# B3zaleel/draco-sharp

Hardware: NVIDIA B200
Metric: decoded points/sec (higher is better)
Workload: dtype i32->f32

## Files before the change

### draco_sharp_b200/csrc/dcb_device.cuh

```cuda
#pragma once
#include <cuda_runtime.h>
#include <stdint.h>

#include "dcb_internal.h"
#include "dcb_kernels.h"

namespace dcb {

__device__ __forceinline__ int32_t zigzag_dec(uint32_t v) {
  return (int32_t)((v >> 1) ^ (0u - (v & 1u)));
}

__device__ __forceinline__ int32_t wrap_original(int32_t pred, int32_t corr, int32_t mn, int32_t mx, int32_t max_diff) {
  pred = pred > mx ? mx : (pred < mn ? mn : pred);
  int32_t o = (int32_t)((uint32_t)pred + (uint32_t)corr);
  if (o > mx)
    o = (int32_t)((uint32_t)o - (uint32_t)max_diff);
  else if (o < mn)
    o = (int32_t)((uint32_t)o + (uint32_t)max_diff);
  return o;
}

__device__ __forceinline__ int32_t wrap_regular(int32_t pred, int32_t corr, int32_t mn, int32_t mx, int32_t max_diff) {
  int32_t o = (int32_t)((uint32_t)pred + (uint32_t)corr);
// ... 203 lines not shown
#define DCB_RING_BYTES 128u
#endif

__device__ __forceinline__ void cp_async16(uint32_t smem_addr, const void *gsrc) {
  asm volatile("cp.async.ca.shared.global [%0], [%1], 16;\n" ::"r"(smem_addr), "l"(gsrc) : "memory");
}
__device__ __forceinline__ void cp_async_commit() { asm volatile("cp.async.commit_group;\n" ::: "memory"); }
template <int N>
__device__ __forceinline__ void cp_async_wait() {
  asm volatile("cp.async.wait_group %0;\n" ::"n"(N) : "memory");
}
__device__ __forceinline__ uint32_t lds_u32(uint32_t a) {
  uint32_t v;
  asm volatile("ld.shared.u32 %0, [%1];\n" : "=r"(v) : "r"(a));
  return v;
}

struct TableGeom {
  uint32_t lut_bytes;
  uint32_t lutb_bytes;
  uint32_t blk_bytes;
  uint32_t ent_bytes;
  uint32_t cap_entries;
  uint32_t cap_exc;
  uint32_t lut_shift;
  uint32_t compact;
  uint32_t zig;
  uint32_t direct_prec;
  uint32_t direct;
};

template <typename T, bool GLOBAL>
struct RansLane {
  uint32_t x;
  uint32_t p1;
  uint32_t L, L8, L16, mask, prec_bits;
  uint32_t lut_base;
  uint32_t lut_mask, lut_sh;
  uint32_t ring;
  uint32_t ent_off;
  uint32_t val_delta;
  uint32_t dprefix;
  uint32_t t_split, a_sh, a_mask, b_base, base_b;
  uint32_t lutb_addr;
  uint32_t blk_addr;
  uint32_t blk_mask;
  uint32_t cum_addr;
  uint32_t n_entries_tab;
  bool split_ok;
  uint32_t max_abs_val;
  uint32_t d_freq, d_off, d_ent;
  const uint8_t *ent0;
  const uint8_t *lut0;
  const uint8_t *arena;
  int64_t end;
  uint32_t p1_init;
  uint32_t off_init;
  int64_t loaded_lo;

  __device__ __forceinline__ uint32_t consumed() const { return p1_init - p1; }
  __device__ __forceinline__ uint32_t bytes_left() const { return off_init - consumed(); }

  template <int MAX_CHUNKS>
  __device__ __forceinline__ void top_up() {
    const int64_t ptr = end - (int64_t)consumed();
    const int64_t floor_lo = ((ptr + 15) & ~15ll) - (int64_t)DCB_RING_BYTES;
#pragma unroll
    for (int k = 0; k < MAX_CHUNKS; ++k) {
      if (loaded_lo - 16 >= floor_lo) {
        loaded_lo -= 16;
        cp_async16(ring | ((uint32_t)loaded_lo & (DCB_RING_BYTES - 1u)), arena + loaded_lo);
      }
    }
    cp_async_commit();
  }

  uint32_t pk_hi, pk_lo, pk_sh;
  __device__ __forceinline__ void prefetch() {
    pk_hi = lds_u32(ring | (p1 & (DCB_RING_BYTES - 4u)));
    pk_lo = lds_u32(ring | ((p1 + DCB_RING_BYTES - 4u) & (DCB_RING_BYTES - 4u)));
    pk_sh = (p1 & 3u) * 8u + 8u;
  }
  __device__ __forceinline__ uint32_t peek() const { return __funnelshift_rc(pk_lo, pk_hi, pk_sh); }

  __device__ __forceinline__ uint32_t lut_load(uint32_t xx) const {
    const uint32_t a = lut_base | ((xx >> lut_sh) & lut_mask);
    if (GLOBAL) return *reinterpret_cast<const T *>(lut0 + a);
    uint32_t v;
    if (sizeof(T) == 2) asm volatile("ld.shared.u16 %0, [%1];\n" : "=r"(v) : "r"(a));
    else asm volatile("ld.shared.u32 %0, [%1];\n" : "=r"(v) : "r"(a));
    return v;
  }

  template <bool CAREFUL, int PROBE>
  __device__ __forceinline__ uint32_t step() {
    const uint32_t v = peek();
    uint32_t sh;
    if (sizeof(T) == 2 && !GLOBAL) {
      const uint32_t sh2 = x < L8 ? 16u : 8u;
      sh = x < L ? sh2 : 0u;
    } else {
      const uint32_t sh3 = x < L16 ? 24u : 16u;
      const uint32_t sh2 = x < L8 ? sh3 : 8u;
      sh = x < L ? sh2 : 0u;
    }
    if (CAREFUL) sh = min(sh, 8u * bytes_left());
    const uint32_t xr = __funnelshift_l(v, x, sh);
    p1 -= sh >> 3;
    prefetch();
    const uint32_t r = xr & mask;
    const uint32_t q = xr >> prec_bits;
    uint32_t o, c0, c1, c2;
    if (PROBE == 2) {
      const uint32_t r2 = r << 1;
      uint32_t f, off;
      asm volatile("ld.shared.u16 %0, [%1];\n" : "=r"(f) : "r"(d_freq + r2));
      asm volatile("ld.shared.u16 %0, [%1];\n" : "=r"(off) : "r"(d_off + r2));
      asm volatile("ld.shared.u16 %0, [%1];\n" : "=r"(o) : "r"(d_ent + r2));
      x = q * f + off;
      return o;
    }
    if (PROBE == 1) {
      const uint32_t a_a = ((xr >> a_sh) & a_mask) | lut_base;
      const uint32_t a_b = (r >> 1) + b_base;
      const uint32_t a = r >= t_split ? a_b : a_a;
      const uint32_t a_k = ((xr >> 5) & blk_mask) | blk_addr;
// ... 113 lines not shown
    const uint32_t rank2 = ca - cum_addr;
    if (rank2 >= 2u * dprefix) {
      int32_t v;
      asm volatile("ld.shared.s16 %0, [%1];\n" : "=r"(v) : "r"(ca + val_delta));
      return v;
    }
    return zigzag_dec(rank2 >> 1);
  }

  __device__ __forceinline__ uint32_t value_at_plain(uint32_t ca, bool compact) const {
    const uint32_t rank2 = ca - cum_addr;
    if (compact && rank2 >= 2u * dprefix) {
      uint32_t v;
      asm volatile("ld.shared.u16 %0, [%1];\n" : "=r"(v) : "r"(ca + val_delta));
      return v;
    }
    return rank2 >> 1;
  }

  __device__ __forceinline__ int32_t value(uint32_t o, bool compact, bool zig) const {
    const uint32_t rank = (o - ent_off) / (uint32_t)sizeof(T);
    if (compact && rank >= dprefix) {
      if (sizeof(T) == 2) {
        return zig ? (int32_t) * reinterpret_cast<const int16_t *>(ent0 + o + val_delta)
                   : (int32_t) * reinterpret_cast<const uint16_t *>(ent0 + o + val_delta);
      }
      return *reinterpret_cast<const int32_t *>(ent0 + o + val_delta);
    }
    return zig ? zigzag_dec(rank) : (int32_t)rank;
  }
  __device__ __forceinline__ uint32_t symbol(uint32_t o, const TableGeom &g) const {
    const int32_t v = value(o, g.compact != 0, g.zig != 0);
    if (!g.zig) return (uint32_t)v;
    return v >= 0 ? ((uint32_t)v << 1) : ((((uint32_t)(-(v + 1))) << 1) | 1u);
  }

  __device__ int init_state(const uint8_t *arena_, const StreamDesc &d) {
    const uint64_t n = d.payload_len;
    if (n < 1) return DCB_ERR_RANS_INIT;
    const uint8_t *p = arena_ + d.payload_off;
    const uint32_t tag = (uint32_t)p[n - 1] >> 6;
    if (n < tag + 1) return DCB_ERR_RANS_INIT;
    uint32_t v = 0;
    for (uint32_t i = 0; i <= tag; ++i) v |= (uint32_t)p[n - 1 - tag + i] << (8 * i);
    v &= (tag == 0) ? 0x3Fu : (tag == 1) ? 0x3FFFu : (tag == 2) ? 0x3FFFFFu : 0x3FFFFFFFu;
    prec_bits = d.prec_bits;
    L = 4u << d.prec_bits;
    L8 = L >> 8;
    L16 = L >> 16;
    mask = (1u << d.prec_bits) - 1u;
    x = v + L;
    if (x >= L * 256u) return DCB_ERR_RANS_INIT;
    off_init = (uint32_t)(n - (tag + 1));
    arena = arena_;
    end = (int64_t)(d.payload_off + off_init);
    p1_init = (uint32_t)end - 1u;
    p1 = p1_init;
    loaded_lo = (end + 15) & ~15ll;
    return DCB_OK;
  }
  __device__ __forceinline__ void init_ring(uint32_t ring_addr) {
    ring = ring_addr;
    top_up<DCB_RING_BYTES / 16>();
    cp_async_wait<0>();
    prefetch();
  }

  __device__ int build(const uint8_t *arena_, const StreamDesc &d, const TableGeom &g, T *ent, uint32_t ent_off_) {
    ent_off = ent_off_;
    lut_sh = g.lut_shift - (sizeof(T) == 2 ? 1u : 2u);
    lut_mask = g.lut_bytes - (uint32_t)sizeof(T);
    split_ok = false;
    T *cum = ent;
    T *val = ent + g.cap_entries + 2u;
    uint64_t pos = d.table_off;
    const uint64_t bend = d.buf_end;
    for (int i = 0; i < 10; ++i) {
      if (pos >= bend) return DCB_ERR_EOF;
      if (!(arena_[pos++] & 0x80)) break;
    }
    const uint32_t ns = d.num_symbols;
    const uint32_t prec = 1u << d.prec_bits;
    if (!g.compact && ns > g.cap_entries) return DCB_ERR_TABLE;
    dprefix = g.compact ? 0xFFFFFFFFu : 0u;
    uint64_t c = 0;
    uint32_t ne = 0;
    bool overflow = false;
    uint32_t last_sym = 0;
    for (uint32_t i = 0; i < ns; ++i) {
      if (pos >= bend) return DCB_ERR_EOF;
      const uint32_t pd = arena_[pos++];
      const uint32_t token = pd & 3u;
      if (token == 3u) {
        const uint32_t off = pd >> 2;
        if (i + off >= ns) return DCB_ERR_TABLE;
        if (!g.compact)
          for (uint32_t j = 0; j <= off; ++j) cum[i + j] = (T)(c > prec ? prec : c);
        i += off;
      } else {
        uint32_t prob = pd >> 2;
        for (uint32_t b = 0; b < token; ++b) {
          if (pos >= bend) return DCB_ERR_EOF;
          prob |= (uint32_t)arena_[pos++] << (8 * (b + 1) - 2);
        }
        if (prob) last_sym = i;
        if (g.compact) {
          if (prob) {
            if (c + prob > prec || ne >= g.cap_entries) overflow = true;
            if (!overflow) {
              if (dprefix == 0xFFFFFFFFu && i != ne) dprefix = ne;
              if (dprefix != 0xFFFFFFFFu) {
// ... 116 lines not shown
    if (g.direct) a = (a + 15u) & ~15u;
    else a = (a + g.lut_bytes - 1u) & ~(g.lut_bytes - 1u);
    l.lut0 = a - base_addr;
    a += lanes * g.lut_bytes;
  } else {
    l.lut0 = 0;
  }
  a = (a + DCB_RING_BYTES - 1u) & ~(DCB_RING_BYTES - 1u);
  l.ring0 = a - base_addr;
  a += lanes * DCB_RING_BYTES;
  l.blk0 = l.lutb0 = a - base_addr;
  if (!table_global && g.lutb_bytes) {
    a = (a + g.blk_bytes - 1u) & ~(g.blk_bytes - 1u);
    l.blk0 = a - base_addr;
    a += lanes * g.blk_bytes;
    l.lutb0 = a - base_addr;
    a += (lanes * g.lutb_bytes + 15u) & ~15u;
  }
  l.ent0 = a - base_addr;
  return l;
}

template <int NCP, typename T, bool TG, bool DUMP, int MODE, int TAB, bool CAREFUL, int PROBE>
__device__ __forceinline__ void decode_entry(RansLane<T, TG> &rl, const TableGeom &g, const PostParams &pp, int32_t *prev,
                                             int32_t *v, int32_t *dptr, uint32_t dump, uint64_t e) {
#pragma unroll
  for (int c = 0; c < NCP; ++c) {
    const uint32_t o = rl.template step<CAREFUL, PROBE>();
    const bool compact = TAB == 0 ? g.compact != 0 : TAB == 2;
    const bool zig = MODE == 0 ? g.zig != 0 : MODE != 3;
    v[c] = rl.value(o, compact, zig);
    if (DUMP && (dump & DCB_DUMP_SYMBOLS)) dptr[e * NCP + c] = (int32_t)rl.symbol(o, g);
  }
  const int recon = recon_of<MODE>(pp);
  if (recon == RECON_DELTA_WRAP) {
#pragma unroll
    for (int c = 0; c < NCP; ++c) {
      prev[c] = wrap_original(prev[c], v[c], pp.mn, pp.mx, pp.max_diff);
      v[c] = prev[c];
    }
  } else if (recon == RECON_DELTA_OCT || recon == RECON_DELTA_OCT_CANON) {
    if (NCP == 2) {
      oct_original(pp.box, recon == RECON_DELTA_OCT_CANON, prev[0], prev[NCP - 1], v[0], v[NCP - 1]);
      v[0] = prev[0];
      v[NCP - 1] = prev[NCP - 1];
    }
  }
  if (DUMP && MODE != 3 && (dump & DCB_DUMP_QINTS)) {
#pragma unroll
    for (int c = 0; c < NCP; ++c) dptr[e * NCP + c] = v[c];
  }
}

template <int NCP, int MODE, bool LAST, int PROBE, bool COMPACT>
__device__ __forceinline__ void lean_sp_group(RansLane<uint16_t, false> &rl, const PostParams &pp, uint8_t *optr, uint32_t g,
                                              int32_t *prev, uint32_t &ca_prev, uint32_t &gate, uint32_t zero) {
  constexpr int kSyms = 4 * NCP;
  float f[kSyms];
  int32_t v[4][NCP];
#pragma unroll
  for (int s = 1; s <= kSyms; ++s) {
    uint32_t ca = 0;
    if (!(LAST && s == kSyms)) {
      const int sp = s % kSyms;
      if (sp % 3 == 0) rl.window_open();
      if (PROBE == 2) ca = (sp % 3 == 0) ? rl.template step_lean_direct<true>(gate, zero) : rl.template step_lean_direct<false>(gate, zero);
      else ca = (sp % 3 == 0) ? rl.template step_lean<true, true>(gate, zero) : rl.template step_lean<false, true>(gate, zero);
      if (sp % 3 == 2 || sp == kSyms - 1) rl.window_close();
    }
    const int c = (s - 1) % NCP;
    const int32_t corr = COMPACT ? rl.value_at(ca_prev) : zigzag_dec((ca_prev - rl.cum_addr) >> 1);
    if (MODE == 3 || MODE == 4) prev[c] = corr;
    else prev[c] = wrap_regular(prev[c], corr, pp.mn, pp.mx, pp.max_diff);
    if (MODE == 1) {
      f[s - 1] = pp.dequant(prev[c], c);
      gate = __float_as_uint(f[s - 1]);
    } else {
      v[(s - 1) / NCP][c] = prev[c];
      gate = (uint32_t)corr;
    }
    ca_prev = ca;
  }
  if (MODE == 1) {
    float4 *o = reinterpret_cast<float4 *>(reinterpret_cast<float *>(optr) + (uint64_t)g * kSyms);
#pragma unroll
    for (int k = 0; k < NCP; ++k) o[k] = make_float4(f[4 * k], f[4 * k + 1], f[4 * k + 2], f[4 * k + 3]);
  } else {
    store_group4<NCP>(pp, store_of<MODE>(pp), dsize_of<MODE>(pp), optr, (uint64_t)g * 4, v);
  }
}

template <bool LAST, int PROBE>
__device__ __forceinline__ void tag_sp_group(RansLane<uint16_t, false> &rl, bool compact, uint32_t *t, uint32_t &ca_prev,
                                             uint32_t &gate, uint32_t zero) {
#pragma unroll
  for (int s = 1; s <= 16; ++s) {
    uint32_t ca = 0;
    if (!(LAST && s == 16)) {
      const int sp = s % 16;
      if (sp % 3 == 0) rl.window_open();
      if (PROBE == 2) ca = (sp % 3 == 0) ? rl.template step_lean_direct<true>(gate, zero) : rl.template step_lean_direct<false>(gate, zero);
      else ca = (sp % 3 == 0) ? rl.template step_lean<true, true>(gate, zero) : rl.template step_lean<false, true>(gate, zero);
      if (sp % 3 == 2 || sp == 15) rl.window_close();
    }
    t[s - 1] = rl.value_at_plain(ca_prev, compact) & 0xFFu;
    gate = t[s - 1];
    ca_prev = ca;
  }
}

template <int PROBE>
__device__ __forceinline__ void run_tags_sp(RansLane<uint16_t, false> &rl, const TableGeom &geom, StreamDesc *dp, uint8_t *aux,
                                            uint32_t zero) {
  const StreamDesc &d = *dp;
  const uint32_t n_entries = d.n_entries;
  const uint32_t ncp = d.ncp;
  const uint64_t avail_bits = (d.buf_end - d.bits_off) * 8ull;
  uint8_t *tags = aux + d.tag_off;
  uint64_t *chunk_bits = reinterpret_cast<uint64_t *>(aux + d.tag_off + (((uint64_t)n_entries + 15ull) & ~15ull));
  const bool compact = geom.compact != 0;
  int status = DCB_OK;
  uint64_t bits = 0;
  uint32_t e = 0;
  if (n_entries >= 16u && rl.bytes_left() >= 48u) {
    rl.window_open();
    uint32_t ca_prev = PROBE == 2 ? rl.template step_lean_direct<true>(0u, zero) : rl.template step_lean<true>();
    uint32_t gate = 0;
    for (;;) {
      const bool last = !(e + 32u <= n_entries && rl.bytes_left() >= 96u);
      if ((e & (DCB_TAG_CHUNK - 1u)) == 0) chunk_bits[e / DCB_TAG_CHUNK] = bits;
      uint32_t t[16];
      if (last) tag_sp_group<true, PROBE>(rl, compact, t, ca_prev, gate, zero);
      else tag_sp_group<false, PROBE>(rl, compact, t, ca_prev, gate, zero);
      uint32_t tmax = 0, tsum = 0;
#pragma unroll
      for (int j = 0; j < 16; ++j) {
        tmax = max(tmax, t[j]);
        tsum += t[j];
      }
      const uint64_t nbits = bits + (uint64_t)tsum * ncp;
      if (tmax > 32u || nbits > avail_bits) {
// ... 45 lines not shown
```

### draco_sharp_b200/csrc/dcb_kernels.cu

```cuda
#include <cuda_runtime.h>
#include <stdint.h>
#include <algorithm>
#include <stdio.h>
#include <stdlib.h>

#include "dcb_device.cuh"
#include "dcb_internal.h"
#include "dcb_kernels.h"
#include "dcb_walk.h"

using namespace dcb;

namespace {

template <int NCP, typename T, bool DUMP, bool TG, int MODE, int TAB, bool SPLIT>
__device__ __forceinline__ void run_tail(RansLane<T, TG> &rl, const TableGeom &geom, const PostParams &pp, uint8_t *optr,
                                         int32_t *dptr, uint32_t dump, uint32_t n_entries, uint32_t g, int32_t *prev);

template <int NCP, typename T, bool DUMP, bool TG, int MODE, int TAB, bool SPLIT>
__device__ __forceinline__ void run_stream(RansLane<T, TG> &rl, const TableGeom &geom, const PostParams &pp, uint8_t *optr,
                                           int32_t *dptr, uint32_t dump, uint32_t n_entries, uint32_t g_min) {
  const int store = store_of<MODE>(pp), dsize = dsize_of<MODE>(pp);
  int32_t prev[NCP];
#pragma unroll
// ... 8 lines not shown
      decode_entry<NCP, T, TG, DUMP, MODE, TAB, false, SPLIT>(rl, geom, pp, prev, v[j], dptr, dump, (uint64_t)g * 4 + j);
    store_group4<NCP>(pp, store, dsize, optr, (uint64_t)g * 4, v);
    rl.template top_up<(kGroupBytes + 15) / 16 + 1>();
    cp_async_wait<1>();
  }
  run_tail<NCP, T, DUMP, TG, MODE, TAB, SPLIT>(rl, geom, pp, optr, dptr, dump, n_entries, g, prev);
}

template <int NCP, typename T, bool DUMP, bool TG, int MODE, int TAB, bool SPLIT>
__device__ __forceinline__ void run_tail(RansLane<T, TG> &rl, const TableGeom &geom, const PostParams &pp, uint8_t *optr,
                                         int32_t *dptr, uint32_t dump, uint32_t n_entries, uint32_t g, int32_t *prev) {
  const int store = store_of<MODE>(pp), dsize = dsize_of<MODE>(pp);
  for (uint32_t e = g * 4u; e < n_entries; ++e) {
    int32_t v[NCP];
    decode_entry<NCP, T, TG, DUMP, MODE, TAB, true, SPLIT>(rl, geom, pp, prev, v, dptr, dump, e);
    store_entry<NCP>(pp, store, dsize, optr, e, v);
    rl.template top_up<(3 * NCP + 15) / 16 + 1>();
    cp_async_wait<0>();
  }
}

template <int NCP, int MODE>
__device__ __forceinline__ void run_stream_lean(RansLane<uint16_t, false> &rl, const TableGeom &geom, const PostParams &pp,
                                                uint8_t *optr, uint32_t n_entries, uint32_t g_min) {
  const int store = store_of<MODE>(pp), dsize = dsize_of<MODE>(pp);
  int32_t prev[NCP];
  const int32_t p0 = 0 > pp.mx ? pp.mx : (0 < pp.mn ? pp.mn : 0);
#pragma unroll
  for (int c = 0; c < NCP; ++c) prev[c] = p0;
  constexpr uint32_t kGroupBytes = 4u * NCP * 3u;
  constexpr int kSyms = 4 * NCP;
  uint32_t g = 0;
  for (; g < g_min; ++g) {
    if (rl.bytes_left() < kGroupBytes) break;
    int32_t v[4][NCP];
#pragma unroll
    for (int s = 0; s < kSyms; ++s) {
      if (s % 3 == 0) rl.window_open();
      const uint32_t ca = (s % 3 == 0) ? rl.template step_lean<true>() : rl.template step_lean<false>();
      if (s % 3 == 2 || s == kSyms - 1) rl.window_close();
      const int32_t corr = rl.value_at(ca);
      const int c = s % NCP;
      prev[c] = wrap_regular(prev[c], corr, pp.mn, pp.mx, pp.max_diff);
      v[s / NCP][c] = prev[c];
    }
    store_group4<NCP>(pp, store, dsize, optr, (uint64_t)g * 4, v);
    rl.template top_up<(kGroupBytes + 15) / 16 + 1>();
    cp_async_wait<1>();
  }
  rl.prefetch();
  run_tail<NCP, uint16_t, false, false, MODE, 2, true>(rl, geom, pp, optr, nullptr, 0u, n_entries, g, prev);
}

template <int NCP, int MODE>
__device__ __forceinline__ void run_stream_lean_sp(RansLane<uint16_t, false> &rl, const TableGeom &geom, const PostParams &pp,
                                                   uint8_t *optr, uint32_t n_entries, uint32_t g_min, uint32_t zero) {
  int32_t prev[NCP];
  const int32_t p0 = 0 > pp.mx ? pp.mx : (0 < pp.mn ? pp.mn : 0);
#pragma unroll
  for (int c = 0; c < NCP; ++c) prev[c] = p0;
  constexpr uint32_t kGroupBytes = 4u * NCP * 3u;
  uint32_t g = 0;
  if (g_min > 0 && rl.bytes_left() >= kGroupBytes) {
    rl.window_open();
    uint32_t ca_prev = rl.template step_lean<true>();
    uint32_t gate = 0;
    while (g + 1 < g_min && rl.bytes_left() >= 2u * kGroupBytes + 4u) {
      lean_sp_group<NCP, MODE, false, 1, true>(rl, pp, optr, g, prev, ca_prev, gate, zero);
      ++g;
      rl.template top_up<(kGroupBytes + 15) / 16 + 1>();
      cp_async_wait<1>();
    }
    lean_sp_group<NCP, MODE, true, 1, true>(rl, pp, optr, g, prev, ca_prev, gate, zero);
    ++g;
    rl.template top_up<(kGroupBytes + 15) / 16 + 1>();
    cp_async_wait<1>();
  }
  rl.prefetch();
  run_tail<NCP, uint16_t, false, false, MODE, 2, true>(rl, geom, pp, optr, nullptr, 0u, n_entries, g, prev);
}

template <int NCP, typename T, bool DUMP, bool TABLE_GLOBAL, int MODE, int TAB>
__global__ void __launch_bounds__(32) rans_raw_fused_kernel(const uint8_t *__restrict__ arena, StreamDesc *streams,
                                                            const uint32_t *__restrict__ order, uint32_t n_streams,
                                                            uint32_t lanes, TableGeom geom, uint8_t *__restrict__ out,
                                                            uint8_t *__restrict__ dbg, uint8_t *__restrict__ aux,
                                                            uint8_t *__restrict__ tab_arena, uint32_t dump) {
  extern __shared__ __align__(16) uint8_t smem[];
  const uint32_t lane = threadIdx.x;
  const uint32_t slot = blockIdx.x * lanes + lane;
  const bool have = lane < lanes && slot < n_streams;
  StreamDesc *dp = have ? &streams[order[slot]] : nullptr;
  const uint32_t smem_base = (uint32_t)__cvta_generic_to_shared(smem);
  const SmemLayout lay = smem_layout(smem_base, lanes, geom, TABLE_GLOBAL);

  RansLane<T, TABLE_GLOBAL> rl;
  uint32_t n_entries = 0;
  T *lut = nullptr, *ent = nullptr;
  uint8_t *lutb = nullptr;
  uint32_t *blk = nullptr;
  bool split_ok = true;
  bool lean_ok = true;
  if (have) {
    const StreamDesc &d = *dp;
    n_entries = d.n_entries;
    if (NCP == 1 && MODE == 0 && d.ncp > 4) n_entries *= d.ncp;
    int status = DCB_OK;
    if (n_entries > 0) {
      uint32_t ent_off;
      if (TABLE_GLOBAL) {
        const uint32_t n_slots = gridDim.x * lanes;
        rl.lut0 = tab_arena;
        rl.ent0 = tab_arena + (size_t)n_slots * geom.lut_bytes;
        rl.lut_base = slot * geom.lut_bytes;
        ent_off = slot * geom.ent_bytes;
        lut = reinterpret_cast<T *>(tab_arena + (size_t)slot * geom.lut_bytes);
        ent = reinterpret_cast<T *>(const_cast<uint8_t *>(rl.ent0) + (size_t)slot * geom.ent_bytes);
      } else {
        rl.lut0 = nullptr;
        rl.ent0 = smem + lay.ent0;
        rl.lut_base = smem_base + lay.lut0 + lane * geom.lut_bytes;
        rl.lutb_addr = smem_base + lay.lutb0 + lane * geom.lutb_bytes;
        rl.blk_addr = smem_base + lay.blk0 + lane * geom.blk_bytes;
        blk = reinterpret_cast<uint32_t *>(smem + lay.blk0 + (size_t)lane * geom.blk_bytes);
        ent_off = lane * geom.ent_bytes;
        rl.cum_addr = smem_base + lay.ent0 + ent_off;
        lut = reinterpret_cast<T *>(smem + lay.lut0 + (size_t)lane * geom.lut_bytes);
        lutb = smem + lay.lutb0 + (size_t)lane * geom.lutb_bytes;
        ent = reinterpret_cast<T *>(smem + lay.ent0 + (size_t)lane * geom.ent_bytes);
      }
      status = rl.build(arena, d, geom, ent, ent_off);
      if (status == DCB_OK) status = rl.init_state(arena, d);
      if (status == DCB_OK) split_ok = rl.split_ok && !(dump & 0x80000000u);
      if (status == DCB_OK) {
        const int64_t md = 1ll + (int64_t)d.xf_b - (int64_t)d.xf_a;
        lean_ok = split_ok && geom.zig != 0 && !(dump & 0x40000000u) &&
                  (MODE == 3 || MODE == 4 ||
                   ((int64_t)rl.max_abs_val < md && d.xf_a >= -(1 << 29) && d.xf_b <= (1 << 29)));
      }
    }
    if (status != DCB_OK) {
      dp->status = status;
      n_entries = 0;
    }
  }
  const bool use_split = __all_sync(0xffffffffu, split_ok);
  const bool use_lean = __all_sync(0xffffffffu, lean_ok);
  uint32_t g_min = n_entries ? (n_entries >> 2) : 0xFFFFFFFFu;
#pragma unroll
  for (int o = 16; o > 0; o >>= 1) g_min = min(g_min, __shfl_xor_sync(0xffffffffu, g_min, o));
  if (n_entries == 0) return;
  rl.fill_lut(geom, lut, lutb, blk, ent, use_split);
  rl.init_ring(smem_base + lay.ring0 + lane * DCB_RING_BYTES);

  PostParams pp;
  pp.load(*dp);
  uint8_t *optr = out + dp->out_off;
  int32_t *dptr = DUMP ? reinterpret_cast<int32_t *>(dbg + dp->dbg_off) : nullptr;
  const bool wide_nc = NCP == 1 && MODE == 0 && dp->ncp > 4;
  if (wide_nc) {
    pp.recon = RECON_NONE;
    dump &= ~(uint32_t)DCB_DUMP_QINTS;
  }
  if (MODE == 3 || MODE == 4 || (MODE == 0 && (pp.recon == RECON_PARA_WRAP || pp.store == STORE_OCT_UNIT || wide_nc))) {
    optr = aux + dp->aux_off;
    if (NCP == 2 && pp.store == STORE_OCT_UNIT) {
      pp.recon = RECON_NONE;
      dump &= ~(uint32_t)DCB_DUMP_QINTS;
    }
    pp.store = STORE_NARROW;
    pp.dsize = 4;
  }
  if constexpr (sizeof(T) == 2 && !TABLE_GLOBAL && !DUMP && MODE >= 1 && MODE <= 4 && TAB == 2) {
    if (use_lean) {
#ifndef DCB_NO_LEAN_SP
      run_stream_lean_sp<NCP, MODE>(rl, geom, pp, optr, n_entries, g_min, blockIdx.y);
      return;
#endif
      if constexpr (MODE == 1 || MODE == 2) {
        run_stream_lean<NCP, MODE>(rl, geom, pp, optr, n_entries, g_min);
        return;
      }
    }
  }
  if (use_split)
    run_stream<NCP, T, DUMP, TABLE_GLOBAL, MODE, TAB, true>(rl, geom, pp, optr, dptr, dump, n_entries, g_min);
  else
    run_stream<NCP, T, DUMP, TABLE_GLOBAL, MODE, TAB, false>(rl, geom, pp, optr, dptr, dump, n_entries, g_min);
}

template <bool SPLIT>
__device__ __forceinline__ void run_tags(RansLane<uint16_t, false> &rl, const TableGeom &geom, StreamDesc *dp, uint8_t *aux) {
  const StreamDesc &d = *dp;
  const uint32_t n_entries = d.n_entries;
  const uint32_t ncp = d.ncp;
  const uint64_t avail_bits = (d.buf_end - d.bits_off) * 8ull;
  uint8_t *tags = aux + d.tag_off;
  uint64_t *chunk_bits = reinterpret_cast<uint64_t *>(aux + d.tag_off + (((uint64_t)n_entries + 15ull) & ~15ull));
  const bool compact = geom.compact != 0;
  int status = DCB_OK;
  uint64_t bits = 0;
  uint32_t e = 0;
  for (; e + 16 <= n_entries; e += 16) {
    if (rl.bytes_left() < 48u) break;
    if ((e & (DCB_TAG_CHUNK - 1u)) == 0) chunk_bits[e / DCB_TAG_CHUNK] = bits;
    uint32_t t[16];
#pragma unroll
    for (int j = 0; j < 16; ++j)
      t[j] = (uint32_t)rl.value(rl.template step<false, SPLIT>(), compact, false) & 0xFFu;
    uint32_t tmax = 0, tsum = 0;
#pragma unroll
    for (int j = 0; j < 16; ++j) {
      tmax = max(tmax, t[j]);
      tsum += t[j];
    }
    const uint64_t nbits = bits + (uint64_t)tsum * ncp;
    if (tmax > 32u || nbits > avail_bits) {
      for (int j = 0; j < 16 && status == DCB_OK; ++j) {
        if (t[j] > 32u) status = DCB_ERR_TAG;
        else {
          bits += (uint64_t)t[j] * ncp;
          if (bits > avail_bits) status = DCB_ERR_EOF;
        }
      }
      break;
    }
    uint4 pk;
    pk.x = t[0] | (t[1] << 8) | (t[2] << 16) | (t[3] << 24);
    pk.y = t[4] | (t[5] << 8) | (t[6] << 16) | (t[7] << 24);
// ... 486 lines not shown
      float x, y, z;
      oct_to_unit(q.x, q.y, scale, x, y, z);
      o[3ull * e] = x;
      o[3ull * e + 1] = y;
      o[3ull * e + 2] = z;
    }
  }
}

__global__ void copy_kernel(const uint8_t *__restrict__ arena, StreamDesc *streams, const uint32_t *__restrict__ order,
                            uint32_t n_streams, uint8_t *__restrict__ out) {
  for (uint32_t si = blockIdx.y; si < n_streams; si += gridDim.y) {
    const StreamDesc &d = streams[order[si]];
    if (d.status != DCB_OK) continue;
    const uint8_t *src = arena + d.raw_off;
    uint8_t *dst = out + d.out_off;
    for (uint64_t i = (uint64_t)blockIdx.x * blockDim.x + threadIdx.x; i < d.out_bytes; i += (uint64_t)gridDim.x * blockDim.x)
      dst[i] = src[i];
  }
}

}

static TableGeom geom_of(const RansLaunch &p) {
  TableGeom g{};
  g.lut_bytes = p.lut_bytes;
  g.lutb_bytes = p.lutb_bytes;
  g.blk_bytes = p.lutb_bytes ? (((1u << p.prec_bits) >> 7) << 2) : 0u;
  if (g.blk_bytes && g.blk_bytes < 16u) g.blk_bytes = 16u;
  g.ent_bytes = p.ent_bytes;
  g.cap_entries = p.cap_entries;
  g.cap_exc = p.cap_exc;
  g.lut_shift = p.lut_shift;
  g.compact = p.compact;
  g.zig = p.zig;
  return g;
}

uint32_t dcb_rans_smem_bytes(const RansLaunch &p, bool table_global) {
  uint32_t b = DCB_RING_BYTES + p.lanes_per_warp * DCB_RING_BYTES;
  if (!table_global && p.direct) return b + 32u + p.lanes_per_warp * (p.lut_bytes + p.ent_bytes);
  if (!table_global) {
    const uint32_t blk = p.lutb_bytes ? std::max(16u, ((1u << p.prec_bits) >> 7) << 2) : 0u;
    b += p.lut_bytes + blk + 16u + p.lanes_per_warp * (p.lut_bytes + p.lutb_bytes + blk + p.ent_bytes);
  }
  return b;
}

static uint32_t no_split_bit() {
  static const uint32_t bit = (getenv("DCB_NO_SPLIT") ? 0x80000000u : 0u) | (getenv("DCB_NO_LEAN") ? 0x40000000u : 0u);
  return bit;
}

template <int NCP, typename T, bool DUMP, bool TG, int MODE, int TAB = 0>
static cudaError_t launch_raw_t(const RansLaunch &p, const DevArenas &a, cudaStream_t st) {
  auto k = rans_raw_fused_kernel<NCP, T, DUMP, TG, MODE, TAB>;
  const uint32_t smem_bytes = dcb_rans_smem_bytes(p, TG);
  if (smem_bytes > 48 * 1024) {
    cudaError_t e = cudaFuncSetAttribute(k, cudaFuncAttributeMaxDynamicSharedMemorySize, (int)smem_bytes);
    if (e != cudaSuccess) return e;
  }
  cudaFuncSetAttribute(k, cudaFuncAttributePreferredSharedMemoryCarveout, (int)cudaSharedmemCarveoutMaxShared);
  const uint32_t grid = (p.n_streams + p.lanes_per_warp - 1) / p.lanes_per_warp;
  k<<<grid, 32, smem_bytes, st>>>(a.in, p.d_streams, p.d_order, p.n_streams, p.lanes_per_warp, geom_of(p), a.out, a.dbg,
                                  a.aux, a.tab, p.dump | no_split_bit());
  return cudaGetLastError();
}

template <int NCP, typename T>
static cudaError_t launch_raw_n(const RansLaunch &p, bool table_global, const DevArenas &a, cudaStream_t st) {
  const bool dump = p.dump != 0;
  if (table_global)
    return dump ? launch_raw_t<NCP, T, true, true, 0>(p, a, st) : launch_raw_t<NCP, T, false, true, 0>(p, a, st);
  return dump ? launch_raw_t<NCP, T, true, false, 0>(p, a, st) : launch_raw_t<NCP, T, false, false, 0>(p, a, st);
}

cudaError_t dcb_launch_rans_raw(const RansLaunch &p, int ncp, bool wide, bool table_global, const DevArenas &a,
                                cudaStream_t st) {
#ifdef DCB_DEV_ONLY_C2
  return launch_raw_t<3, uint16_t, false, false, 1, 2>(p, a, st);
#else
  if (!wide && !table_global && !p.dump) {
#define DCB_SPEC(M, N)                                                                           \
  if (p.mode == M && ncp == N)                                                                   \
    return p.compact ? launch_raw_t<N, uint16_t, false, false, M, 2>(p, a, st)                   \
                     : launch_raw_t<N, uint16_t, false, false, M, 1>(p, a, st);
    DCB_SPEC(1, 3)
    DCB_SPEC(1, 2)
    DCB_SPEC(2, 3)
    DCB_SPEC(2, 4)
    DCB_SPEC(3, 2)
    DCB_SPEC(4, 3)
    DCB_SPEC(4, 2)
#undef DCB_SPEC
  }
#define DCB_CASE(N)                                                       \
  case N:                                                                 \
    return wide ? launch_raw_n<N, uint32_t>(p, table_global, a, st)       \
                : launch_raw_n<N, uint16_t>(p, table_global, a, st);
  switch (ncp) {
    DCB_CASE(1)
    DCB_CASE(2)
    DCB_CASE(3)
    DCB_CASE(4)
    default:
      return cudaErrorInvalidValue;
  }
#undef DCB_CASE
#endif
}

cudaError_t dcb_launch_rans_tag(const RansLaunch &p, const DevArenas &a, cudaStream_t st) {
  const uint32_t smem_bytes = dcb_rans_smem_bytes(p, false);
  if (smem_bytes > 48 * 1024) {
    cudaError_t e = cudaFuncSetAttribute(rans_tag_kernel, cudaFuncAttributeMaxDynamicSharedMemorySize, (int)smem_bytes);
    if (e != cudaSuccess) return e;
  }
  cudaFuncSetAttribute(rans_tag_kernel, cudaFuncAttributePreferredSharedMemoryCarveout, (int)cudaSharedmemCarveoutMaxShared);
  const uint32_t grid = (p.n_streams + p.lanes_per_warp - 1) / p.lanes_per_warp;
  rans_tag_kernel<<<grid, 32, smem_bytes, st>>>(a.in, p.d_streams, p.d_order, p.n_streams, p.lanes_per_warp, geom_of(p),
                                                a.aux);
  return cudaGetLastError();
}

cudaError_t dcb_launch_wide_post(StreamDesc *d_streams, const uint32_t *d_order, uint32_t n, uint32_t dump, const DevArenas &a,
                                 cudaStream_t st) {
  if (n == 0) return cudaSuccess;
  const uint32_t grid = (n + 31) / 32;
  if (dump)
    wide_post_kernel<true><<<grid, 32, 0, st>>>(a.in, d_streams, d_order, n, a.out, a.dbg, a.aux, dump);
  else
    wide_post_kernel<false><<<grid, 32, 0, st>>>(a.in, d_streams, d_order, n, a.out, a.dbg, a.aux, dump);
  return cudaGetLastError();
}

cudaError_t dcb_launch_resolve(const DevArenas &a, BufWalk *d_walks, const uint32_t *d_list, uint32_t n,
                               StreamDesc *d_streams, cudaStream_t st) {
  if (n == 0) return cudaSuccess;
  resolve_kernel<<<(n + 63) / 64, 64, 0, st>>>(a.in, d_walks, d_list, n, d_streams);
// ... 91 lines not shown
```

### draco_sharp_b200/csrc/dcb_rans_pc.cu

```cuda
#include <cuda_runtime.h>
#include <stdint.h>
#include <stdlib.h>
#include <algorithm>

#include "dcb_device.cuh"
#include "dcb_internal.h"
#include "dcb_kernels.h"

using namespace dcb;

namespace {

constexpr uint32_t kStages = DCB_PC_STAGES;
constexpr uint32_t kRowBytes = DCB_PC_ROW_BYTES;

struct LaneHand {
  uint32_t dprefix;
  int32_t active;
  int32_t prev[4];
  int32_t status;
  uint32_t e;
  uint32_t ne;
  uint32_t fused;
  uint64_t bits;
// ... 153 lines not shown
    if (!slot_free) mbar_wait(ctl.empty(s), par ^ 1u);
    __syncwarp();
    if (lane == 0) {
      sts_u32(ctl.flag(s), 1u);
      mbar_arrive(ctl.full(s));
    }
  }
  return g;
}

struct ValMap {
  const uint8_t *ent0;
  uint32_t ent_off, dprefix, val_delta;
  __device__ __forceinline__ int32_t value(uint32_t o, bool compact, bool zig) const {
    const uint32_t rank = (o - ent_off) >> 1;
    if (compact && rank >= dprefix) {
      return zig ? (int32_t) * reinterpret_cast<const int16_t *>(ent0 + o + val_delta)
                 : (int32_t) * reinterpret_cast<const uint16_t *>(ent0 + o + val_delta);
    }
    return zig ? zigzag_dec(rank) : (int32_t)rank;
  }
  __device__ __forceinline__ uint32_t symbol(uint32_t o, bool compact, bool zig) const {
    const int32_t v = value(o, compact, zig);
    if (!zig) return (uint32_t)v;
    return v >= 0 ? ((uint32_t)v << 1) : ((((uint32_t)(-(v + 1))) << 1) | 1u);
  }
};

template <int NCP, int MODE>
__device__ __forceinline__ void redirect_post(PostParams &pp, uint32_t &dump, uint8_t *&optr, uint8_t *aux, const StreamDesc &d) {
  if (MODE == 3 || MODE == 4 || (MODE == 0 && (pp.recon == RECON_PARA_WRAP || pp.store == STORE_OCT_UNIT))) {
    optr = aux + d.aux_off;
    if (NCP == 2 && pp.store == STORE_OCT_UNIT) {
      pp.recon = RECON_NONE;
      dump &= ~(uint32_t)DCB_DUMP_QINTS;
    }
    pp.store = STORE_NARROW;
    pp.dsize = 4;
  }
}

template <int NCP, int MODE, bool COMPACT>
__device__ __forceinline__ uint32_t fused_direct_loop(RansLane<uint16_t, false> &rl, const PostParams &pp, uint8_t *optr,
                                                      uint32_t g_min, int32_t *prev, uint32_t zero) {
  constexpr uint32_t kGroupBytes = 4u * NCP * 3u;
  uint32_t g = 0;
  if (g_min != 0xFFFFFFFFu && g_min > 0 && rl.bytes_left() >= kGroupBytes) {
    rl.window_open();
    uint32_t ca_prev = rl.template step_lean_direct<true>(0u, zero);
    uint32_t gate = 0;
    while (g + 1 < g_min && rl.bytes_left() >= 2u * kGroupBytes + 4u) {
      lean_sp_group<NCP, MODE, false, 2, COMPACT>(rl, pp, optr, g, prev, ca_prev, gate, zero);
      ++g;
      rl.template top_up<(kGroupBytes + 15) / 16 + 1>();
      cp_async_wait<1>();
    }
    lean_sp_group<NCP, MODE, true, 2, COMPACT>(rl, pp, optr, g, prev, ca_prev, gate, zero);
    ++g;
    rl.template top_up<(kGroupBytes + 15) / 16 + 1>();
    cp_async_wait<1>();
  }
  rl.prefetch();
  return g;
}

template <int NCP, bool DUMP, int MODE, int TAB>
__global__ void __launch_bounds__(384) rans_raw_pc_kernel(const uint8_t *__restrict__ arena, StreamDesc *streams,
                                                          const uint32_t *__restrict__ order, uint32_t n_streams,
                                                          uint32_t lanes, uint32_t pairs, TableGeom geom, PcGeom pc,
                                                          uint8_t *__restrict__ out, uint8_t *__restrict__ dbg,
                                                          uint8_t *__restrict__ aux, uint32_t dump) {
  extern __shared__ __align__(16) uint8_t smem[];
  typedef uint16_t T;
  constexpr int kSym = 4 * NCP;
  const uint32_t lane = threadIdx.x & 31u, warp = threadIdx.x >> 5;
  uint32_t pair, role;
  warp_role(warp, pairs, pair, role);
  uint8_t *slice = smem + (size_t)pair * pc.slice_bytes;
  const uint32_t slice_addr = smem_u32(slice);
  const uint32_t q_addr = slice_addr + pc.q_off;
  const PairCtl ctl{slice_addr + pc.ctl_off};
  if (role == 0 && lane == 0) {
#pragma unroll
    for (uint32_t i = 0; i < kNumBarriers; ++i) mbar_init(ctl.base + 8u * i, i == 2u * kStages + 2u ? 2u : 1u);
  }
  __syncthreads();
  if (role == 2u) return;
  const uint32_t slot = (blockIdx.x * pairs + pair) * lanes + lane;
  const bool have = lane < lanes && slot < n_streams;
  StreamDesc *dp = have ? &streams[order[slot]] : nullptr;
  LaneHand *hand = reinterpret_cast<LaneHand *>(slice + pc.hand_off) + (have ? lane : 0u);
  const SmemLayout lay = smem_layout(slice_addr, lanes, geom, false);
  const bool compact = TAB == 0 ? geom.compact != 0 : TAB == 2;
  const bool zig = MODE == 0 ? geom.zig != 0 : MODE != 3;

  if (role == 0) {
    RansLane<T, false> rl;
    uint32_t n_entries = 0;
    bool split_ok = true;
    T *lut = nullptr, *ent = nullptr;
    uint8_t *lutb = nullptr;
    uint32_t *blk = nullptr;
    rl.dprefix = 0;
    if (have) {
      const StreamDesc &d = *dp;
      n_entries = d.n_entries;
      int status = DCB_OK;
      if (n_entries > 0) {
        rl.lut0 = nullptr;
        rl.ent0 = slice + lay.ent0;
        rl.lut_base = slice_addr + lay.lut0 + lane * geom.lut_bytes;
        rl.lutb_addr = slice_addr + lay.lutb0 + lane * geom.lutb_bytes;
// ... 466 lines not shown
```

Measured before the change: 38.63 billion.

## Batch lean rANS decode into multi-quad groups with warp-uniform trip counts

Rewrites the ring top-up to use 32-bit offsets and predicated cp.async instead of 64-bit arithmetic and branches. The lean single-pass decoder now handles E quads per group (default 8), calling top_up once per quad and moving the cp.async wait inside the window-open point. The outer loop runs a warp-uniform count computed with ballot and reduce_min, so lanes stay converged and per-iteration checks are fewer. In exchange the kernel carries more template instantiations and a tighter byte margin, which makes the ring refill safety harder to verify.

```diff
diff --git a/draco_sharp_b200/csrc/dcb_device.cuh b/draco_sharp_b200/csrc/dcb_device.cuh
--- a/draco_sharp_b200/csrc/dcb_device.cuh
+++ b/draco_sharp_b200/csrc/dcb_device.cuh
@@ -279,26 +279,26 @@
   uint32_t d_freq, d_off, d_ent;
   const uint8_t *ent0;
   const uint8_t *lut0;
-  const uint8_t *arena;
-  int64_t end;
+  const uint8_t *lo_ptr;
+  uint32_t lo;
   uint32_t p1_init;
   uint32_t off_init;
-  int64_t loaded_lo;
 
   __device__ __forceinline__ uint32_t consumed() const { return p1_init - p1; }
   __device__ __forceinline__ uint32_t bytes_left() const { return off_init - consumed(); }
 
   template <int MAX_CHUNKS>
   __device__ __forceinline__ void top_up() {
-    const int64_t ptr = end - (int64_t)consumed();
-    const int64_t floor_lo = ((ptr + 15) & ~15ll) - (int64_t)DCB_RING_BYTES;
+    const uint32_t floor_lo = ((p1 + 16u) & ~15u) - DCB_RING_BYTES;
+    const uint32_t n = min((lo - floor_lo) >> 4, (uint32_t)MAX_CHUNKS);
 #pragma unroll
     for (int k = 0; k < MAX_CHUNKS; ++k) {
-      if (loaded_lo - 16 >= floor_lo) {
-        loaded_lo -= 16;
-        cp_async16(ring | ((uint32_t)loaded_lo & (DCB_RING_BYTES - 1u)), arena + loaded_lo);
-      }
-    }
+      asm volatile("{\n .reg .pred p;\n setp.gt.u32 p, %2, %3;\n @p cp.async.ca.shared.global [%0], [%1], 16;\n}\n"
+                   ::"r"(ring | ((lo - 16u * (k + 1)) & (DCB_RING_BYTES - 1u))), "l"(lo_ptr - 16 * (k + 1)), "r"(n),
+                   "r"((uint32_t)k) : "memory");
+    }
+    lo -= n << 4;
+    lo_ptr -= n << 4;
     cp_async_commit();
   }
 
@@ -518,11 +518,11 @@
     x = v + L;
     if (x >= L * 256u) return DCB_ERR_RANS_INIT;
     off_init = (uint32_t)(n - (tag + 1));
-    arena = arena_;
-    end = (int64_t)(d.payload_off + off_init);
+    const uint64_t end = d.payload_off + off_init;
     p1_init = (uint32_t)end - 1u;
     p1 = p1_init;
-    loaded_lo = (end + 15) & ~15ll;
+    lo_ptr = arena_ + ((end + 15u) & ~15ull);
+    lo = ((uint32_t)end + 15u) & ~15u;
     return DCB_OK;
   }
   __device__ __forceinline__ void init_ring(uint32_t ring_addr) {
@@ -745,41 +745,52 @@
   }
 }
 
-template <int NCP, int MODE, bool LAST, int PROBE, bool COMPACT>
+template <int NCP, int MODE, bool LAST, int PROBE, bool COMPACT, int E = 4>
 __device__ __forceinline__ void lean_sp_group(RansLane<uint16_t, false> &rl, const PostParams &pp, uint8_t *optr, uint32_t g,
                                               int32_t *prev, uint32_t &ca_prev, uint32_t &gate, uint32_t zero) {
-  constexpr int kSyms = 4 * NCP;
-  float f[kSyms];
-  int32_t v[4][NCP];
-#pragma unroll
-  for (int s = 1; s <= kSyms; ++s) {
-    uint32_t ca = 0;
-    if (!(LAST && s == kSyms)) {
-      const int sp = s % kSyms;
-      if (sp % 3 == 0) rl.window_open();
-      if (PROBE == 2) ca = (sp % 3 == 0) ? rl.template step_lean_direct<true>(gate, zero) : rl.template step_lean_direct<false>(gate, zero);
-      else ca = (sp % 3 == 0) ? rl.template step_lean<true, true>(gate, zero) : rl.template step_lean<false, true>(gate, zero);
-      if (sp % 3 == 2 || sp == kSyms - 1) rl.window_close();
-    }
-    const int c = (s - 1) % NCP;
-    const int32_t corr = COMPACT ? rl.value_at(ca_prev) : zigzag_dec((ca_prev - rl.cum_addr) >> 1);
-    if (MODE == 3 || MODE == 4) prev[c] = corr;
-    else prev[c] = wrap_regular(prev[c], corr, pp.mn, pp.mx, pp.max_diff);
+  static_assert(E % 4 == 0 && (!LAST || E == 4), "groups of whole quads; the LAST group is one quad");
+  constexpr int kQuad = 4 * NCP;
+  constexpr int kSyms = E * NCP;
+#pragma unroll
+  for (int qd = 0; qd < E / 4; ++qd) {
+    float f[kQuad];
+    int32_t v[4][NCP];
+#pragma unroll
+    for (int t = 1; t <= kQuad; ++t) {
+      const int s = qd * kQuad + t;
+      uint32_t ca = 0;
+      if (!(LAST && s == kSyms)) {
+        const int sp = s % kSyms;
+        if (sp % 3 == 0) {
+          if (sp != 0 && sp <= qd * kQuad + 3) cp_async_wait<1>();
+          rl.window_open();
+        }
+        if (PROBE == 2) ca = (sp % 3 == 0) ? rl.template step_lean_direct<true>(gate, zero) : rl.template step_lean_direct<false>(gate, zero);
+        else ca = (sp % 3 == 0) ? rl.template step_lean<true, true>(gate, zero) : rl.template step_lean<false, true>(gate, zero);
+        if (sp % 3 == 2 || sp == kSyms - 1) rl.window_close();
+      }
+      const int c = (t - 1) % NCP;
+      const int32_t corr = COMPACT ? rl.value_at(ca_prev) : zigzag_dec((ca_prev - rl.cum_addr) >> 1);
+      if (MODE == 3 || MODE == 4) prev[c] = corr;
+      else prev[c] = wrap_regular(prev[c], corr, pp.mn, pp.mx, pp.max_diff);
+      if (MODE == 1) {
+        f[t - 1] = pp.dequant(prev[c], c);
+        gate = __float_as_uint(f[t - 1]);
+      } else {
+        v[(t - 1) / NCP][c] = prev[c];
+        gate = (uint32_t)corr;
+      }
+      ca_prev = ca;
+    }
+    const uint32_t gq = g + (uint32_t)qd;
     if (MODE == 1) {
-      f[s - 1] = pp.dequant(prev[c], c);
-      gate = __float_as_uint(f[s - 1]);
+      float4 *o = reinterpret_cast<float4 *>(reinterpret_cast<float *>(optr) + (uint64_t)gq * kQuad);
+#pragma unroll
+      for (int k = 0; k < NCP; ++k) o[k] = make_float4(f[4 * k], f[4 * k + 1], f[4 * k + 2], f[4 * k + 3]);
     } else {
-      v[(s - 1) / NCP][c] = prev[c];
-      gate = (uint32_t)corr;
-    }
-    ca_prev = ca;
-  }
-  if (MODE == 1) {
-    float4 *o = reinterpret_cast<float4 *>(reinterpret_cast<float *>(optr) + (uint64_t)g * kSyms);
-#pragma unroll
-    for (int k = 0; k < NCP; ++k) o[k] = make_float4(f[4 * k], f[4 * k + 1], f[4 * k + 2], f[4 * k + 3]);
-  } else {
-    store_group4<NCP>(pp, store_of<MODE>(pp), dsize_of<MODE>(pp), optr, (uint64_t)g * 4, v);
+      store_group4<NCP>(pp, store_of<MODE>(pp), dsize_of<MODE>(pp), optr, (uint64_t)gq * 4, v);
+    }
+    rl.template top_up<(4 * NCP * 3 + 15) / 16 + 1>();
   }
 }
 
diff --git a/draco_sharp_b200/csrc/dcb_kernels.cu b/draco_sharp_b200/csrc/dcb_kernels.cu
--- a/draco_sharp_b200/csrc/dcb_kernels.cu
+++ b/draco_sharp_b200/csrc/dcb_kernels.cu
@@ -84,35 +84,44 @@
   run_tail<NCP, uint16_t, false, false, MODE, 2, true>(rl, geom, pp, optr, nullptr, 0u, n_entries, g, prev);
 }
 
-template <int NCP, int MODE>
+template <int NCP, int MODE, int E>
 __device__ __forceinline__ void run_stream_lean_sp(RansLane<uint16_t, false> &rl, const TableGeom &geom, const PostParams &pp,
-                                                   uint8_t *optr, uint32_t n_entries, uint32_t g_min, uint32_t zero) {
+                                                   uint8_t *optr, uint32_t n_entries, uint32_t g_min, uint32_t zero,
+                                                   uint32_t live) {
   int32_t prev[NCP];
   const int32_t p0 = 0 > pp.mx ? pp.mx : (0 < pp.mn ? pp.mn : 0);
 #pragma unroll
   for (int c = 0; c < NCP; ++c) prev[c] = p0;
-  constexpr uint32_t kGroupBytes = 4u * NCP * 3u;
+  constexpr uint32_t kQuads = E / 4;
+  constexpr uint32_t kMaxGroupBytes = 2u * E * NCP;
+  constexpr uint32_t kMargin = 2u * 4u * NCP;
   uint32_t g = 0;
-  if (g_min > 0 && rl.bytes_left() >= kGroupBytes) {
+  const bool fast = g_min > 0 && rl.bytes_left() >= kMargin;
+  uint32_t run = __ballot_sync(live, fast);
+  if (fast) {
     rl.window_open();
     uint32_t ca_prev = rl.template step_lean<true>();
     uint32_t gate = 0;
-    while (g + 1 < g_min && rl.bytes_left() >= 2u * kGroupBytes + 4u) {
-      lean_sp_group<NCP, MODE, false, 1, true>(rl, pp, optr, g, prev, ca_prev, gate, zero);
-      ++g;
-      rl.template top_up<(kGroupBytes + 15) / 16 + 1>();
-      cp_async_wait<1>();
+    for (;;) {
+      const uint32_t by_bytes = rl.bytes_left() >= kMargin + kMaxGroupBytes ? (rl.bytes_left() - kMargin) / kMaxGroupBytes : 0u;
+      const uint32_t mine = min(by_bytes, (g_min - 1u - g) / kQuads);
+      run = __ballot_sync(run, mine > 0);
+      if (mine == 0) break;
+      const uint32_t n = __reduce_min_sync(run, mine);
+      for (uint32_t i = 0; i < n; ++i) {
+        lean_sp_group<NCP, MODE, false, 1, true, E>(rl, pp, optr, g, prev, ca_prev, gate, zero);
+        g += kQuads;
+      }
     }
     lean_sp_group<NCP, MODE, true, 1, true>(rl, pp, optr, g, prev, ca_prev, gate, zero);
     ++g;
-    rl.template top_up<(kGroupBytes + 15) / 16 + 1>();
     cp_async_wait<1>();
   }
   rl.prefetch();
   run_tail<NCP, uint16_t, false, false, MODE, 2, true>(rl, geom, pp, optr, nullptr, 0u, n_entries, g, prev);
 }
 
-template <int NCP, typename T, bool DUMP, bool TABLE_GLOBAL, int MODE, int TAB>
+template <int NCP, typename T, bool DUMP, bool TABLE_GLOBAL, int MODE, int TAB, int E>
 __global__ void __launch_bounds__(32) rans_raw_fused_kernel(const uint8_t *__restrict__ arena, StreamDesc *streams,
                                                             const uint32_t *__restrict__ order, uint32_t n_streams,
                                                             uint32_t lanes, TableGeom geom, uint8_t *__restrict__ out,
@@ -181,6 +190,7 @@
   uint32_t g_min = n_entries ? (n_entries >> 2) : 0xFFFFFFFFu;
 #pragma unroll
   for (int o = 16; o > 0; o >>= 1) g_min = min(g_min, __shfl_xor_sync(0xffffffffu, g_min, o));
+  const uint32_t live = __ballot_sync(0xffffffffu, n_entries != 0);
   if (n_entries == 0) return;
   rl.fill_lut(geom, lut, lutb, blk, ent, use_split);
   rl.init_ring(smem_base + lay.ring0 + lane * DCB_RING_BYTES);
@@ -206,7 +216,7 @@
   if constexpr (sizeof(T) == 2 && !TABLE_GLOBAL && !DUMP && MODE >= 1 && MODE <= 4 && TAB == 2) {
     if (use_lean) {
 #ifndef DCB_NO_LEAN_SP
-      run_stream_lean_sp<NCP, MODE>(rl, geom, pp, optr, n_entries, g_min, blockIdx.y);
+      run_stream_lean_sp<NCP, MODE, E>(rl, geom, pp, optr, n_entries, g_min, blockIdx.y, live);
       return;
 #endif
       if constexpr (MODE == 1 || MODE == 2) {
@@ -799,9 +809,19 @@
   return bit;
 }
 
-template <int NCP, typename T, bool DUMP, bool TG, int MODE, int TAB = 0>
+constexpr int kLeanGroup = 8;
+static int lean_group() {
+  static const int e = [] {
+    const char *v = getenv("DCB_LEAN_GROUP");
+    const int x = v ? atoi(v) : 0;
+    return (x == 4 || x == 8 || x == 16) ? x : kLeanGroup;
+  }();
+  return e;
+}
+
+template <int NCP, typename T, bool DUMP, bool TG, int MODE, int TAB = 0, int E = 4>
 static cudaError_t launch_raw_t(const RansLaunch &p, const DevArenas &a, cudaStream_t st) {
-  auto k = rans_raw_fused_kernel<NCP, T, DUMP, TG, MODE, TAB>;
+  auto k = rans_raw_fused_kernel<NCP, T, DUMP, TG, MODE, TAB, E>;
   const uint32_t smem_bytes = dcb_rans_smem_bytes(p, TG);
   if (smem_bytes > 48 * 1024) {
     cudaError_t e = cudaFuncSetAttribute(k, cudaFuncAttributeMaxDynamicSharedMemorySize, (int)smem_bytes);
@@ -825,13 +845,18 @@
 cudaError_t dcb_launch_rans_raw(const RansLaunch &p, int ncp, bool wide, bool table_global, const DevArenas &a,
                                 cudaStream_t st) {
 #ifdef DCB_DEV_ONLY_C2
-  return launch_raw_t<3, uint16_t, false, false, 1, 2>(p, a, st);
+  return launch_raw_t<3, uint16_t, false, false, 1, 2, kLeanGroup>(p, a, st);
 #else
   if (!wide && !table_global && !p.dump) {
 #define DCB_SPEC(M, N)                                                                           \
-  if (p.mode == M && ncp == N)                                                                   \
-    return p.compact ? launch_raw_t<N, uint16_t, false, false, M, 2>(p, a, st)                   \
-                     : launch_raw_t<N, uint16_t, false, false, M, 1>(p, a, st);
+  if (p.mode == M && ncp == N) {                                                                 \
+    if (!p.compact) return launch_raw_t<N, uint16_t, false, false, M, 1>(p, a, st);              \
+    switch (lean_group()) {                                                                      \
+      case 4: return launch_raw_t<N, uint16_t, false, false, M, 2, 4>(p, a, st);                 \
+      case 16: return launch_raw_t<N, uint16_t, false, false, M, 2, 16>(p, a, st);               \
+      default: return launch_raw_t<N, uint16_t, false, false, M, 2, 8>(p, a, st);                \
+    }                                                                                            \
+  }
     DCB_SPEC(1, 3)
     DCB_SPEC(1, 2)
     DCB_SPEC(2, 3)
diff --git a/draco_sharp_b200/csrc/dcb_rans_pc.cu b/draco_sharp_b200/csrc/dcb_rans_pc.cu
--- a/draco_sharp_b200/csrc/dcb_rans_pc.cu
+++ b/draco_sharp_b200/csrc/dcb_rans_pc.cu
@@ -229,12 +229,9 @@
     while (g + 1 < g_min && rl.bytes_left() >= 2u * kGroupBytes + 4u) {
       lean_sp_group<NCP, MODE, false, 2, COMPACT>(rl, pp, optr, g, prev, ca_prev, gate, zero);
       ++g;
-      rl.template top_up<(kGroupBytes + 15) / 16 + 1>();
-      cp_async_wait<1>();
     }
     lean_sp_group<NCP, MODE, true, 2, COMPACT>(rl, pp, optr, g, prev, ca_prev, gate, zero);
     ++g;
-    rl.template top_up<(kGroupBytes + 15) / 16 + 1>();
     cp_async_wait<1>();
   }
   rl.prefetch();
```

Result: faster. 41.45 billion (median of 6 runs) (+7.3%).
